# KTH-RPL/cloth-splatting

Hardware: AMD Instinct MI355X
Metric: rasterizer fwd+bwd rendered Mpix/s (scene_1, 800x800) (higher is better)
Workload: dtype f32

## Files before the change

cloth-splatting_amd/csrc/csplat_raster.hip:

```cpp
#include "csplat_common.h"

#include <atomic>
#include <cstring>
#include <chrono>
#include <mutex>
#include <type_traits>

namespace {

constexpr float NEAR_Z = 0.2f;

__device__ constexpr float SH_C0 = 0.28209479177387814f;
__device__ constexpr float SH_C1 = 0.4886025119029199f;
__device__ constexpr float SH_C2[5] = {1.0925484305920792f, -1.0925484305920792f, 0.31539156525252005f,
                                       -1.0925484305920792f, 0.5462742152960396f};
__device__ constexpr float SH_C3[7] = {-0.5900435899266435f, 2.890611442640554f, -0.4570457994644658f,
                                       0.3731763325901154f, -0.4570457994644658f, 1.445305721320277f,
                                       -0.5900435899266435f};

struct Geom {
    float *depth;
    float2 *xy;
    float4 *conic_opacity;
    float *rgb;
// ... 217 lines not shown

    g.depth[i] = depth;
    radii[i] = rad;
    g.xy[i] = make_float2(px, py);
    g.conic_opacity[i] = co;
#pragma unroll
    for (int k = 0; k < 3; k++) g.rgb[3 * i + k] = rgb[k];
#pragma unroll
    for (int k = 0; k < 6; k++) g.cov3D[6 * i + k] = c6[k];
    g.clamped[i] = clampbits;
    g.tiles_touched[i] = touched;
    g.cut2[i] = cut;
    g.pack[3 * (size_t)i] = make_float4(px, py, co.x, co.y);
    g.pack[3 * (size_t)i + 1] = make_float4(co.z, co.w, rgb[0], rgb[1]);
    g.pack[3 * (size_t)i + 2] = make_float4(rgb[2], depth, cut, 0.f);
}

template <bool STAGE>
__global__ __launch_bounds__(256) void k_preprocess(int P, int D, int M, const float *__restrict__ means3D,
                                                     const float *__restrict__ shs,
                                                     const float *__restrict__ colors_precomp,
                                                     const float *__restrict__ opacities,
                                                     const float *__restrict__ scales, float scale_mod,
                                                     const float *__restrict__ rotations,
                                                     const float *__restrict__ cov3D_precomp, Cam cam, Geom g,
                                                     int32_t *__restrict__ radii, int nocull) {
    __shared__ float s_shrows[STAGE ? 256 * SH_ROW : 1];
    if (STAGE) {
        const int base = blockIdx.x * 256;
        stage_sh_rows<256>(shs + (size_t)base * 48, min(256, P - base), s_shrows);
        __syncthreads();
    }
    preprocess_body<STAGE>(P, D, M, means3D, shs, colors_precomp, opacities, scales, scale_mod, rotations, cov3D_precomp, cam, g, radii,
                           nocull, s_shrows, (int)(blockIdx.x * blockDim.x + threadIdx.x), (int)threadIdx.x);
}

constexpr int K1_MAX_VIEWS = 8;
struct K1View {
    const float *means3D, *rotations;
    Cam cam;
    Geom g;
    int32_t *radii;
    uint32_t *table, *info, *mailbox;
    int2 *ranges;
    uint32_t tag;
};
struct K1Table { int n; K1View v[K1_MAX_VIEWS]; };

constexpr int K1V_G = 64;
template <bool STAGE>
__global__ __launch_bounds__(256) void k_preprocess_views(int P, int D, int M, const float *__restrict__ shs,
                                                           const float *__restrict__ opacities,
                                                           const float *__restrict__ scales, float scale_mod, K1Table tab,
                                                           int nocull) {
    __shared__ float s_shrows[STAGE ? K1V_G * SH_ROW : 1];
    const int base = blockIdx.x * K1V_G;
    if (STAGE) {
        stage_sh_rows<256>(shs + (size_t)base * 48, min(K1V_G, P - base), s_shrows);
        __syncthreads();
    }
    const int lane = threadIdx.x & 63;
    for (int vi = threadIdx.x >> 6; vi < tab.n; vi += 4) {
        const K1View &w = tab.v[vi];
        preprocess_body<STAGE>(P, D, M, w.means3D, shs, nullptr, opacities, scales, scale_mod, w.rotations, nullptr, w.cam, w.g, w.radii, nocull,
                               s_shrows, base + lane, lane);
    }
}

__global__ __launch_bounds__(256) void k_emit_keys(int P, const float2 *__restrict__ xy, const float *__restrict__ depth,
                                                    const uint32_t *__restrict__ offsets,
                                                    const int32_t *__restrict__ radii, Cam cam,
                                                    uint64_t *__restrict__ keys, uint32_t *__restrict__ ids) {
    const int i = blockIdx.x * blockDim.x + threadIdx.x;
    if (i >= P) return;
    const int rad = radii[i];
    if (rad <= 0) return;
    uint32_t off = (i == 0) ? 0u : offsets[i - 1];
    const float2 p = xy[i];
    int minx, miny, maxx, maxy;
    tile_rect(p.x, p.y, rad, cam, minx, miny, maxx, maxy);
    const uint32_t dbits = __float_as_uint(depth[i]);
    for (int y = miny; y < maxy; y++)
        for (int x = minx; x < maxx; x++) {
            keys[off] = ((uint64_t)(uint32_t)(y * cam.gx + x) << 32) | dbits;
            ids[off] = (uint32_t)i;
            off++;
        }
}

__global__ __launch_bounds__(256) void k_tile_ranges(int64_t R, const uint64_t *__restrict__ keys, int2 *__restrict__ ranges) {
    const int64_t i = (int64_t)blockIdx.x * blockDim.x + threadIdx.x;
    if (i >= R) return;
    const uint32_t t = (uint32_t)(keys[i] >> 32);
    if (i == 0) ranges[t].x = 0;
    else {
        const uint32_t tp = (uint32_t)(keys[i - 1] >> 32);
        if (tp != t) { ranges[tp].y = (int)i; ranges[t].x = (int)i; }
    }
    if (i == R - 1) ranges[t].y = (int)R;
}

constexpr int BUCKET_CAP = 8192;
constexpr int BUCKET_TILES = 12288;
constexpr int BUCKET_G = 1024;

__device__ __forceinline__ void tile_count_body(int P, int tiles, const float2 *__restrict__ xy,
                                                const int32_t *__restrict__ radii, const Cam &cam,
                                                uint32_t *__restrict__ table) {
    extern __shared__ uint32_t s_hist[];
    for (int t = threadIdx.x; t < tiles; t += BUCKET_G) s_hist[t] = 0u;
    __syncthreads();
    const int i = blockIdx.x * BUCKET_G + threadIdx.x;
    if (i < P) {
        const int rad = radii[i];
        if (rad > 0) {
            const float2 p = xy[i];
            int minx, miny, maxx, maxy;
            tile_rect(p.x, p.y, rad, cam, minx, miny, maxx, maxy);
            for (int y = miny; y < maxy; y++)
                for (int x = minx; x < maxx; x++) atomicAdd(&s_hist[y * cam.gx + x], 1u);
        }
    }
    __syncthreads();
    uint32_t *row = table + (size_t)blockIdx.x * tiles;
    for (int t = threadIdx.x; t < tiles; t += BUCKET_G) row[t] = s_hist[t];
}
__global__ __launch_bounds__(BUCKET_G) void k_tile_count(int P, int tiles, const float2 *__restrict__ xy,
                                                          const int32_t *__restrict__ radii, Cam cam,
                                                          uint32_t *__restrict__ table) {
    tile_count_body(P, tiles, xy, radii, cam, table);
}
__global__ __launch_bounds__(BUCKET_G) void k_tile_count_views(int P, int tiles, K1Table tab) {
    const K1View &w = tab.v[blockIdx.y];
    tile_count_body(P, tiles, w.g.xy, w.radii, w.cam, w.table);
}

__device__ __forceinline__ void tile_colscan_body(int tiles, int nb, uint32_t *__restrict__ table, uint32_t *__restrict__ cnt) {
    const int t = blockIdx.x * 256 + threadIdx.x;
    if (t >= tiles) return;
    uint32_t run = 0;
    int b = 0;
    for (; b + 8 <= nb; b += 8) {
        uint32_t v[8];
#pragma unroll
        for (int u = 0; u < 8; u++) v[u] = table[(size_t)(b + u) * tiles + t];
#pragma unroll
        for (int u = 0; u < 8; u++) { table[(size_t)(b + u) * tiles + t] = run; run += v[u]; }
    }
    for (; b < nb; b++) { const uint32_t v = table[(size_t)b * tiles + t]; table[(size_t)b * tiles + t] = run; run += v; }
    cnt[t] = run;
}
__global__ __launch_bounds__(256) void k_tile_colscan(int tiles, int nb, uint32_t *__restrict__ table, uint32_t *__restrict__ cnt) {
    tile_colscan_body(tiles, nb, table, cnt);
}
__global__ __launch_bounds__(256) void k_tile_colscan_views(int tiles, int nb, K1Table tab) {
    uint32_t *table = tab.v[blockIdx.y].table;
    tile_colscan_body(tiles, nb, table, table + (size_t)nb * tiles);
}

constexpr int INFO_BUSY = 64;
constexpr int LPT_BINS = 512;
__device__ __forceinline__ void tile_scan_body(int tiles, const uint32_t *__restrict__ cnt, int2 *__restrict__ ranges,
                                               uint32_t *__restrict__ info, volatile uint32_t *mailbox, uint32_t tag) {
    __shared__ unsigned long long s_w[17];
    __shared__ uint32_t s_max[16];
    const int lane = threadIdx.x & 63, w = threadIdx.x >> 6;
    unsigned long long carry = 0ull;
    uint32_t mx = 0;
    uint32_t *busy = info + INFO_BUSY;
    for (int base = 0; base < tiles; base += 1024) {
        const int t = base + threadIdx.x;
        const uint32_t c = t < tiles ? cnt[t] : 0u;
        mx = max(mx, c);
        const unsigned long long v0 = (unsigned long long)c | ((unsigned long long)(c ? 1u : 0u) << 32);
        unsigned long long inc = v0;
#pragma unroll
        for (int d = 1; d < 64; d <<= 1) { const unsigned long long o = __shfl_up(inc, d, 64); if (lane >= d) inc += o; }
        if (lane == 63) s_w[w] = inc;
        __syncthreads();
        if (w == 0) {
            unsigned long long v = lane < 16 ? s_w[lane] : 0ull, vi = v;
#pragma unroll
            for (int d = 1; d < 16; d <<= 1) { const unsigned long long o = __shfl_up(vi, d, 64); if (lane >= d) vi += o; }
            if (lane < 16) s_w[lane] = vi - v;
            if (lane == 15) s_w[16] = vi;
        }
        __syncthreads();
        const unsigned long long exl = carry + s_w[w] + inc - v0;
        const uint32_t ex = (uint32_t)exl;
        if (t < tiles) {
            ranges[t] = c ? make_int2((int)ex, (int)(ex + c)) : make_int2(0, 0);
            if (c) busy[1 + (uint32_t)(exl >> 32)] = (uint32_t)t;
            else busy[tiles + 4 + tiles - 1 - (t - (int)(uint32_t)(exl >> 32))] = (uint32_t)t;
        }
        carry += s_w[16];
        __syncthreads();
    }
    {
        __shared__ uint32_t s_bin[LPT_BINS + 1];
        const uint32_t nbusy = (uint32_t)(carry >> 32);
        uint32_t *lpt = busy + tiles + 4;
        for (int i = threadIdx.x; i <= LPT_BINS; i += 1024) s_bin[i] = 0u;
        __syncthreads();
        for (uint32_t i = threadIdx.x; i < nbusy; i += 1024) {
            const uint32_t c = cnt[busy[1 + i]];
            atomicAdd(&s_bin[LPT_BINS - 1 - min(c >> 4, (uint32_t)(LPT_BINS - 1))], 1u);
        }
        __syncthreads();
        if (w == 0) {
            uint32_t v[LPT_BINS / 64], run = 0;
// ... 43 lines not shown

__device__ __forceinline__ void emit_bucket_body(int P, int tiles, const float2 *__restrict__ xy,
                                                 const float *__restrict__ depth, const int32_t *__restrict__ radii,
                                                 const Cam &cam, const uint32_t *__restrict__ table,
                                                 const int2 *__restrict__ ranges, uint64_t *__restrict__ comp) {
    extern __shared__ uint32_t s_base[];
    const uint32_t *row = table + (size_t)blockIdx.x * tiles;
    for (int t = threadIdx.x; t < tiles; t += BUCKET_G) s_base[t] = (uint32_t)ranges[t].x + row[t];
    __syncthreads();
    const int i = blockIdx.x * BUCKET_G + threadIdx.x;
    if (i >= P) return;
    const int rad = radii[i];
    if (rad <= 0) return;
    const float2 p = xy[i];
    int minx, miny, maxx, maxy;
    tile_rect(p.x, p.y, rad, cam, minx, miny, maxx, maxy);
    const uint64_t v = ((uint64_t)__float_as_uint(depth[i]) << 32) | (uint32_t)i;
    for (int y = miny; y < maxy; y++)
        for (int x = minx; x < maxx; x++) comp[atomicAdd(&s_base[y * cam.gx + x], 1u)] = v;
}
__global__ __launch_bounds__(BUCKET_G) void k_emit_bucket(int P, int tiles, const float2 *__restrict__ xy,
                                                           const float *__restrict__ depth, const int32_t *__restrict__ radii,
                                                           Cam cam, const uint32_t *__restrict__ table,
                                                           const int2 *__restrict__ ranges, uint64_t *__restrict__ comp) {
    emit_bucket_body(P, tiles, xy, depth, radii, cam, table, ranges, comp);
}

constexpr int P2_MAX_VIEWS = 8;
struct P2View {
    Geom g;
    Cam cam;
    const int32_t *radii;
    const uint32_t *table;
    int2 *ranges;
    uint64_t *keys_u, *keys_sorted;
    uint32_t *ids_sorted;
    int *seg_offset, *slot_tile;
    float4 *ckpt;
    uint16_t *mask16;
    unsigned long long *bbits;
    unsigned long long *bmask;
    float4 *recA, *recB;
    float2 *recC;
    const float *bg;
    float *final_T;
    uint32_t *n_contrib;
    float *out_color, *out_depth;
    uint32_t R;
    const uint32_t *info;
    uint32_t Lcap;
    uint32_t Bcap;
    int spec;
};
struct P2Table { P2View v[P2_MAX_VIEWS]; uint32_t *valid; int nviews; };
__device__ __forceinline__ bool p2_live(const P2View &w) { return !w.spec || (w.info[0] - 1u < w.R && w.info[1] <= w.Lcap && w.info[2] <= w.Bcap); }
__device__ __forceinline__ void seg_plan_body(int tiles, const int2 *__restrict__ ranges, int *__restrict__ seg_offset,
                                              int *__restrict__ slot_tile);
__global__ __launch_bounds__(BUCKET_G) void k_emit_bucket_views(int P, int tiles, P2Table tab) {
    const P2View &w = tab.v[blockIdx.y];
    if (!p2_live(w)) return;
    if (blockIdx.x == gridDim.x - 1) { seg_plan_body(tiles, w.ranges, w.seg_offset, w.slot_tile); return; }
    emit_bucket_body(P, tiles, w.g.xy, w.g.depth, w.radii, w.cam, w.table, w.ranges, w.keys_u);
}

constexpr int TSORT_THREADS = 1024;
constexpr int TSORT_WAVES = TSORT_THREADS / 64;
constexpr int TSORT_ITEMS = BUCKET_CAP / TSORT_THREADS;
constexpr int TSORT_NB = 4 * TSORT_THREADS;
constexpr int TSORT_GRID = 512;
constexpr int TSORT_LONG = 64;
constexpr int TSORT_WORDS = TSORT_NB + 4 + 256 + 8 + 2 + 2 + TSORT_WAVES + 2;
__host__ __device__ inline size_t tsort_lds_bytes(int longest) {
    const int items = (longest > 0 ? longest : 1) + TSORT_THREADS - 1;
    return (size_t)(items / TSORT_THREADS) * TSORT_THREADS * 8 + (size_t)TSORT_WORDS * 4;
}

__device__ __forceinline__ void tile_sort_body(const int2 *__restrict__ ranges, const uint64_t *__restrict__ comp,
                                               uint64_t *__restrict__ keys_sorted,
                                               uint32_t *__restrict__ ids_sorted, int mode, int tile) {
    extern __shared__ uint64_t s_key[];
    const int2 r = ranges[tile];
    const int n = r.y - r.x;
    if (n <= 0) return;
    const int skip_byte3 = mode & 1;
    const int items = (n + TSORT_THREADS - 1) / TSORT_THREADS;
    uint32_t *s_cnt = reinterpret_cast<uint32_t *>(s_key + (size_t)items * TSORT_THREADS);
    uint32_t *s_dig = s_cnt + TSORT_NB + 4;
    const int lane = threadIdx.x & 63, w = threadIdx.x >> 6;
    const int wbase = w * items * 64;
    const uint64_t lt = (1ull << lane) - 1ull;
    uint64_t key[TSORT_ITEMS];
    uint32_t rank[TSORT_ITEMS];
#pragma unroll
    for (int i = 0; i < TSORT_ITEMS; i++) {
        const int idx = wbase + i * 64 + lane;
        key[i] = (i < items && idx < n) ? comp[r.x + idx] : ~0ull;
    }
    uint32_t *s_diff = s_dig + 264;
    uint32_t *s_mm = s_diff + 2;
    uint32_t *s_wtot = s_mm + 2;
    const uint64_t hi = (uint64_t)(uint32_t)tile << 32;
    if (!(mode & 2)) {
        uint32_t dmin = ~0u, dmax = 0u;
#pragma unroll
        for (int i = 0; i < TSORT_ITEMS; i++) {
            const int idx = wbase + i * 64 + lane;
            if (i < items && idx < n) { const uint32_t d = (uint32_t)(key[i] >> 32); dmin = min(dmin, d); dmax = max(dmax, d); }
// ... 589 lines not shown
        for (int o = 1; o < 16; o <<= 1) m = max(m, (uint32_t)__shfl_xor((int)m, o, 64));
        if (lane == 0) reinterpret_cast<uint32_t *>(seg_offset)[tiles + 1 + tile * 16 + blk] = m;
    }
    if (inside && r == 0) {
        final_T[pix] = T;
        n_contrib[pix] = last;
        const size_t HW = (size_t)H * W;
        out_color[pix] = C0 + T * bg[0];
        out_color[HW + pix] = C1 + T * bg[1];
        out_color[2 * HW + pix] = C2 + T * bg[2];
        out_depth[pix] = Dp;
    }
}
template <int CTRL>
__device__ __forceinline__ float dpp_add(float v) {
    return v + __int_as_float(__builtin_amdgcn_update_dpp(0, __float_as_int(v), CTRL, 0xF, 0xF, false));
}
#define CSPLAT_ROW_SCAN4(OP, N, FIRST, a, b, c, d)                                                                                  \
    asm(FIRST "v_" OP "_f32_dpp %0, %0, %0 row_shr:" #N " row_mask:0xf bank_mask:0xf\n\t"                                          \
              "v_" OP "_f32_dpp %1, %1, %1 row_shr:" #N " row_mask:0xf bank_mask:0xf\n\t"                                          \
              "v_" OP "_f32_dpp %2, %2, %2 row_shr:" #N " row_mask:0xf bank_mask:0xf\n\t"                                          \
              "v_" OP "_f32_dpp %3, %3, %3 row_shr:" #N " row_mask:0xf bank_mask:0xf"                                               \
        : "+v"(a), "+v"(b), "+v"(c), "+v"(d))
__device__ __forceinline__ void row_scan4_mul(float (&x)[4]) {
    CSPLAT_ROW_SCAN4("mul", 1, "s_nop 1\n\t", x[0], x[1], x[2], x[3]);
    CSPLAT_ROW_SCAN4("mul", 2, "", x[0], x[1], x[2], x[3]);
    CSPLAT_ROW_SCAN4("mul", 4, "", x[0], x[1], x[2], x[3]);
    CSPLAT_ROW_SCAN4("mul", 8, "", x[0], x[1], x[2], x[3]);
}
__device__ __forceinline__ void row_scan4_add(float (&x)[4]) {
    CSPLAT_ROW_SCAN4("add", 1, "s_nop 1\n\t", x[0], x[1], x[2], x[3]);
    CSPLAT_ROW_SCAN4("add", 2, "", x[0], x[1], x[2], x[3]);
    CSPLAT_ROW_SCAN4("add", 4, "", x[0], x[1], x[2], x[3]);
    CSPLAT_ROW_SCAN4("add", 8, "", x[0], x[1], x[2], x[3]);
}
__device__ __forceinline__ void row_scan4_min(float (&x)[4]) {
    CSPLAT_ROW_SCAN4("min", 1, "s_nop 1\n\t", x[0], x[1], x[2], x[3]);
    CSPLAT_ROW_SCAN4("min", 2, "", x[0], x[1], x[2], x[3]);
    CSPLAT_ROW_SCAN4("min", 4, "", x[0], x[1], x[2], x[3]);
    CSPLAT_ROW_SCAN4("min", 8, "", x[0], x[1], x[2], x[3]);
}
__device__ __forceinline__ float row_total(float v) {
    v = dpp_add<0xB1>(v); v = dpp_add<0x4E>(v); v = dpp_add<0x141>(v); v = dpp_add<0x140>(v);
    return v;
}
__device__ __forceinline__ void composite_fwd16_body(int tiles, int W, int H, int gx, const int2 *__restrict__ ranges,
                                                     const uint16_t *__restrict__ mask16, const float4 *__restrict__ recA,
                                                     const float4 *__restrict__ recB, const float2 *__restrict__ recC,
                                                     uint32_t null_rec, const float *__restrict__ bg,
                                                     int *seg_offset, float4 *__restrict__ ckpt,
                                                     float *__restrict__ final_T, uint32_t *__restrict__ n_contrib,
                                                     float *__restrict__ out_color, float *__restrict__ out_depth,
                                                     unsigned long long *__restrict__ bbits,
                                                     const unsigned long long *__restrict__ bmask,
                                                     const uint32_t *__restrict__ order = nullptr) {
    __shared__ int s_ring[RING16];
    __shared__ uint32_t s_hit[SEG / 32];
    const int wg = blockIdx.x;
    const int item = ((wg >> 7) << 3) + (wg & 7), blk = (wg >> 3) & 15;
    if (item >= tiles) return;
    const int tile = order ? (int)order[item] : item;
    const int lane = threadIdx.x, sv = lane & 15, q = lane >> 4;
    const int px0 = (tile % gx) * CSPLAT_TILE + (blk & 3) * 4;
    const int py = (tile / gx) * CSPLAT_TILE + (blk >> 2) * 4 + q;
    const float fy = (float)py;
    const int2 range = ranges[tile];
    const int n = range.y - range.x;
    const uint32_t rx = (uint32_t)range.x;
    __shared__ float s_Tend[16];
    bool inside[4];
    unsigned long long m_done[4];
    float T[4], C0[4], C1[4], C2[4], Dp[4], fx[4];
    uint32_t last[4];
#pragma unroll
    for (int j = 0; j < 4; j++) {
        inside[j] = px0 + j < W && py < H;
        m_done[j] = __builtin_amdgcn_ballot_w64(!inside[j]);
        T[j] = inside[j] ? 1.f : 0.f; C0[j] = C1[j] = C2[j] = Dp[j] = 0.f;
        last[j] = 0u;
        fx[j] = (float)(px0 + j);
    }
    int seg0 = 0, seg_written = -1;
    if (n > 0 && (m_done[0] & m_done[1] & m_done[2] & m_done[3]) != ~0ull) {
        seg0 = seg_offset[tile];
        WordStreamT<16, RING16> st;
        st.start(bmask, rx, n, blk, lane, s_ring);
        if (lane < SEG / 32) s_hit[lane] = 0u;
        auto fetch = [&](Trip &t, int k) -> bool {
            const bool ok = st.group(k, sv, t.pos);
            const uint32_t ri = t.pos >= 0 ? rx + (uint32_t)t.pos : null_rec;
            t.a = recA[ri]; t.b = recB[ri]; t.c = recC[ri];
            return ok;
        };
        auto process = [&](const Trip &t) {
            const int seg = __builtin_amdgcn_readfirstlane(t.pos) / SEG;
            if (seg != seg_written) {
#pragma unroll
                for (int j = 0; j < 4; j++) {
                    const float t0 = row_total(C0[j]), t1 = row_total(C1[j]), t2 = row_total(C2[j]);
                    if (sv == 0)
                        for (int s_ = seg_written + 1; s_ <= seg; s_++)
                            ckpt[(size_t)(seg0 + s_) * 256 + blk * 16 + q * 4 + j] = make_float4(T[j], t0, t1, t2);
                    C0[j] = sv == 0 ? t0 : 0.f; C1[j] = sv == 0 ? t1 : 0.f; C2[j] = sv == 0 ? t2 : 0.f;
                }
                if (seg_written >= 0) bbits_flush(s_hit, bbits, (size_t)(seg0 + seg_written), blk, lane);
                for (int s_ = seg_written + 1; s_ < seg; s_++) bbits_zero(bbits, (size_t)(seg0 + s_), blk, lane);
                seg_written = seg;
            }
            const float dy = t.a.y - fy;
            float al[4], inc[4];
            unsigned long long m_live[4];
// ... 81 lines not shown
#pragma unroll
    for (int j = 0; j < 4; j++)
        if (inside[j] && __builtin_amdgcn_inverse_ballot_w64(m_done[j])) T[j] = s_Tend[q * 4 + j];
    uint32_t hi_ = 0u;
#pragma unroll
    for (int j = 0; j < 4; j++) {
        C0[j] = row_total(C0[j]); C1[j] = row_total(C1[j]); C2[j] = row_total(C2[j]); Dp[j] = row_total(Dp[j]);
        uint32_t m = last[j];
#pragma unroll
        for (int o = 1; o < 16; o <<= 1) m = max(m, (uint32_t)__shfl_xor((int)m, o, 64));
        last[j] = m;
        hi_ = max(hi_, inside[j] ? m : 0u);
    }
    {
#pragma unroll
        for (int o = 16; o < 64; o <<= 1) hi_ = max(hi_, (uint32_t)__shfl_xor((int)hi_, o, 64));
        if (lane == 0) reinterpret_cast<uint32_t *>(seg_offset)[tiles + 1 + tile * 16 + blk] = hi_;
    }
    if (sv < 4) {
        const size_t HW = (size_t)H * W;
        float t_ = T[0], c0 = C0[0], c1 = C1[0], c2 = C2[0], dp = Dp[0];
        uint32_t la = last[0];
        bool in_ = inside[0];
#pragma unroll
        for (int j = 1; j < 4; j++)
            if (sv == j) { t_ = T[j]; c0 = C0[j]; c1 = C1[j]; c2 = C2[j]; dp = Dp[j]; la = last[j]; in_ = inside[j]; }
        if (in_) {
            const int pix = py * W + px0 + sv;
            final_T[pix] = t_;
            n_contrib[pix] = la;
            out_color[pix] = c0 + t_ * bg[0];
            out_color[HW + pix] = c1 + t_ * bg[1];
            out_color[2 * HW + pix] = c2 + t_ * bg[2];
            out_depth[pix] = dp;
        }
    }
    if (seg_written >= 0) bbits_flush(s_hit, bbits, (size_t)(seg0 + seg_written), blk, lane);
}
template <bool ROWS>
__global__ __launch_bounds__(64) void k_composite_fwd(int tiles, int W, int H, int gx, const int2 *__restrict__ ranges,
                                                       const uint16_t *__restrict__ mask16, const float4 *__restrict__ recA,
                                                       const float4 *__restrict__ recB, const float2 *__restrict__ recC,
                                                       uint32_t null_rec, const float *__restrict__ bg,
                                                       int *seg_offset, float4 *__restrict__ ckpt,
                                                       float *__restrict__ final_T, uint32_t *__restrict__ n_contrib,
                                                       float *__restrict__ out_color, float *__restrict__ out_depth,
                                                       unsigned long long *__restrict__ bbits,
                                                       const unsigned long long *__restrict__ bmask) {
    if (ROWS)
        composite_fwd_body(tiles, W, H, gx, ranges, mask16, recA, recB, recC, null_rec, bg, seg_offset, ckpt, final_T, n_contrib, out_color,
                           out_depth, (int)blockIdx.x, bbits);
    else
        composite_fwd16_body(tiles, W, H, gx, ranges, mask16, recA, recB, recC, null_rec, bg, seg_offset, ckpt, final_T, n_contrib, out_color,
                             out_depth, bbits, bmask);
}
constexpr int K6_EXTRA = 256;
__device__ __forceinline__ void paint_empty_tiles(int tiles, int W, int H, int gx, const uint32_t *__restrict__ order, int busy_grid,
                                                  const float *__restrict__ bg, int *seg_offset, float *__restrict__ final_T,
                                                  uint32_t *__restrict__ n_contrib, float *__restrict__ out_color,
                                                  float *__restrict__ out_depth) {
    const int lane = threadIdx.x;
    const size_t HW = (size_t)H * W;
    const float b0 = bg[0], b1 = bg[1], b2 = bg[2];
    uint32_t *blk_hi = reinterpret_cast<uint32_t *>(seg_offset) + tiles + 1;
    for (int pos = (busy_grid >> 7 << 3) + ((int)blockIdx.x - busy_grid); pos < tiles; pos += (int)gridDim.x - busy_grid) {
        const int tile = (int)order[pos];
        if (lane < 16) blk_hi[tile * 16 + lane] = 0u;
#pragma unroll
        for (int q = 0; q < 4; q++) {
            const int px = (tile % gx) * CSPLAT_TILE + (lane & 15), py = (tile / gx) * CSPLAT_TILE + 4 * q + (lane >> 4);
            if (px < W && py < H) {
                const int pix = py * W + px;
                final_T[pix] = 1.f;
                n_contrib[pix] = 0u;
                out_color[pix] = b0; out_color[HW + pix] = b1; out_color[2 * HW + pix] = b2;
                out_depth[pix] = 0.f;
            }
        }
    }
}
template <bool ROWS>
__global__ __launch_bounds__(64) __attribute__((amdgpu_waves_per_eu(5))) void k_composite_fwd_views(int tiles, int W, int H, P2Table tab, int busy_grid) {
    if (tab.valid && blockIdx.x == 0 && blockIdx.y == 0 && threadIdx.x == 0) {
        bool ok = true;
        for (int i = 0; i < tab.nviews; i++) ok = ok && p2_live(tab.v[i]);
        *tab.valid = ok ? 1u : 0u;
    }
    const P2View &w = tab.v[blockIdx.y];
    if (!p2_live(w)) return;
    const uint32_t *order = w.info + INFO_BUSY + tiles + 4;
    if ((int)blockIdx.x >= busy_grid) {
        paint_empty_tiles(tiles, W, H, w.cam.gx, order, busy_grid, w.bg, w.seg_offset, w.final_T, w.n_contrib, w.out_color, w.out_depth);
        return;
    }
    if (ROWS)
        composite_fwd_body(tiles, W, H, w.cam.gx, w.ranges, w.mask16, w.recA, w.recB, w.recC, w.R, w.bg, w.seg_offset, w.ckpt, w.final_T,
                           w.n_contrib, w.out_color, w.out_depth, (int)blockIdx.x, w.bbits, order);
    else
        composite_fwd16_body(tiles, W, H, w.cam.gx, w.ranges, w.mask16, w.recA, w.recB, w.recC, w.R, w.bg, w.seg_offset, w.ckpt, w.final_T,
                             w.n_contrib, w.out_color, w.out_depth, w.bbits, w.bmask, order);
}

constexpr int ACC_STRIDE = 16;

#define CSPLAT_ROWMASK_OP(OP, dst, src0, src1, RM)                                                                                  \
    asm("s_nop 1\n\tv_" OP "_f32_dpp %0, %1, %2 quad_perm:[0,1,2,3] row_mask:" RM " bank_mask:0xf" : "+v"(dst) : "v"(src0), "v"(src1))
__device__ __forceinline__ void rows_scan_mul(float f, float Tin, float &Tr, float &Tout) {
    const auto s16 = __builtin_amdgcn_permlane16_swap(__float_as_uint(f), __float_as_uint(f), false, false);
    const float ev = __uint_as_float(s16[0]), od = __uint_as_float(s16[1]);
    const float pr = ev * od;
    const auto s32 = __builtin_amdgcn_permlane32_swap(__float_as_uint(pr), __float_as_uint(pr), false, false);
    const float lo = __uint_as_float(s32[0]), hi = __uint_as_float(s32[1]);
    float base = Tin;
    CSPLAT_ROWMASK_OP("mul", base, lo, Tin, "0xc");
    Tr = base;
    CSPLAT_ROWMASK_OP("mul", Tr, ev, base, "0xa");
    Tout = (Tin * lo) * hi;
}
__device__ __forceinline__ void rows_scan_add(float g, float Sin, float &Sr, float &Sout) {
    const auto s16 = __builtin_amdgcn_permlane16_swap(__float_as_uint(g), __float_as_uint(g), false, false);
    const float ev = __uint_as_float(s16[0]), od = __uint_as_float(s16[1]);
    const float pr = ev + od;
    const auto s32 = __builtin_amdgcn_permlane32_swap(__float_as_uint(pr), __float_as_uint(pr), false, false);
    const float lo = __uint_as_float(s32[0]), hi = __uint_as_float(s32[1]);
    float base = Sin;
    CSPLAT_ROWMASK_OP("add", base, lo, Sin, "0xc");
    float incl = ev;
    CSPLAT_ROWMASK_OP("add", incl, od, ev, "0xa");
    Sr = base + incl;
    Sout = (Sin + lo) + hi;
}
#ifndef CSPLAT_K7X
#define CSPLAT_K7X 0
#endif
constexpr int RING7 = SEG;
template <bool DET, bool DEPTH = false, bool FEAT = false>
__device__ __forceinline__ void composite_bwd_body(int tiles, int W, int H, int gx, const int2 *__restrict__ ranges,
                                                   const uint32_t *__restrict__ ids_sorted,
                                                   const unsigned long long *__restrict__ bbits, const float4 *__restrict__ recA,
                                                   const float4 *__restrict__ recB, const float2 *__restrict__ recC,
                                                   uint32_t null_rec, const int *__restrict__ seg_offset,
                                                   const int *__restrict__ slot_tile, const float4 *__restrict__ ckpt,
                                                   const float *__restrict__ final_T, const uint32_t *__restrict__ n_contrib,
                                                   const float *__restrict__ out_color, const float *__restrict__ dL_dpix,
                                                   float *__restrict__ acc, float *__restrict__ det,
                                                   unsigned long long *stamp = nullptr, int wg = (int)blockIdx.x,
                                                   const float *__restrict__ dL_ddepth = nullptr, const float *__restrict__ dpart = nullptr,
                                                   const float *__restrict__ features = nullptr, int nf = 0,
                                                   const float *__restrict__ dL_dfeat = nullptr, const float *__restrict__ dL_dalpha = nullptr,
                                                   const float *__restrict__ wpart = nullptr) {
    static_assert(!FEAT || DEPTH, "the feature path is instantiated on the depth path");
    constexpr int DS = FEAT ? 16 : (DEPTH ? 10 : 9);
    using TT = std::conditional_t<FEAT, TripF, Trip>;
// ... 1318 lines not shown
        if (stage)
            k_preprocess<true><<<cdiv(P, 256), 256, 0, s>>>(P, t.D, t.M, t.means3D, t.shs, t.colors_precomp, t.opacities, t.scales,
                                                             t.scale_modifier, t.rotations, t.cov3D_precomp, t.cam, t.g, t.radii, nocull_mode());
        else
            k_preprocess<false><<<cdiv(P, 256), 256, 0, s>>>(P, t.D, t.M, t.means3D, t.shs, t.colors_precomp, t.opacities, t.scales,
                                                              t.scale_modifier, t.rotations, t.cov3D_precomp, t.cam, t.g, t.radii, nocull_mode());
        LAUNCH_CHECK();
    }
    if (t.can_bucket) {
        ProfScope ps(PROF_K2, s);
        if (P > 0) {
            k_tile_count<<<nb, BUCKET_G, (size_t)tiles * 4, s>>>(P, tiles, t.g.xy, t.radii, t.cam, t.table);
            LAUNCH_CHECK();
        } else {
            HIP_TRY(hipMemsetAsync(t.table, 0, (size_t)nb * tiles * 4, s));
        }
        uint32_t *tile_cnt = t.table + (size_t)nb * tiles;
        k_tile_colscan<<<cdiv(tiles, 256), 256, 0, s>>>(tiles, nb, t.table, tile_cnt);
        LAUNCH_CHECK();
        k_tile_scan<<<1, 1024, 0, s>>>(tiles, tile_cnt, t.ranges, t.info, t.mb_dev, t.tag);
        LAUNCH_CHECK();
    }
    return 0;
}

static bool begin_views_compatible(int V, const int *tk) {
    if (V < 1 || V > K1_MAX_VIEWS || (g_debug_flags & 512u)) return false;
    const FwdTicket &a = g_tickets[tk[0]];
    if (a.P <= 0 || !a.can_bucket || !a.shs || a.colors_precomp || a.cov3D_precomp || !a.scales || !a.rotations) return false;
    for (int i = 1; i < V; i++) {
        const FwdTicket &w = g_tickets[tk[i]];
        if (w.P != a.P || w.D != a.D || w.M != a.M || w.W != a.W || w.H != a.H || w.shs != a.shs || w.opacities != a.opacities ||
            w.scales != a.scales || w.scale_modifier != a.scale_modifier || w.colors_precomp || w.cov3D_precomp || !w.rotations ||
            !w.can_bucket)
            return false;
    }
    return true;
}
static int begin_launch_views(int V, const int *tk, hipStream_t join) {
    const FwdTicket &a = g_tickets[tk[0]];
    const int P = a.P, tiles = a.tiles, nb = a.nb;
    K1Table tab;
    tab.n = V;
    for (int i = 0; i < V; i++) {
        const FwdTicket &t = g_tickets[tk[i]];
        K1View &k = tab.v[i];
        k.means3D = t.means3D; k.rotations = t.rotations; k.cam = t.cam; k.g = t.g; k.radii = t.radii; k.table = t.table;
        k.info = t.info; k.mailbox = t.mb_dev; k.ranges = t.ranges; k.tag = t.tag;
    }
    {
        ProfScope ps(PROF_K1, join);
        const bool stage = a.M == 16 && ((uintptr_t)a.shs & 15u) == 0;
        if (stage)
            k_preprocess_views<true><<<cdiv(P, K1V_G), 256, 0, join>>>(P, a.D, a.M, a.shs, a.opacities, a.scales, a.scale_modifier, tab,
                                                                     nocull_mode());
        else
            k_preprocess_views<false><<<cdiv(P, K1V_G), 256, 0, join>>>(P, a.D, a.M, a.shs, a.opacities, a.scales, a.scale_modifier, tab,
                                                                      nocull_mode());
        LAUNCH_CHECK();
    }
    {
        ProfScope ps(PROF_K2, join);
        k_tile_count_views<<<dim3(nb, V), BUCKET_G, (size_t)tiles * 4, join>>>(P, tiles, tab);
        LAUNCH_CHECK();
        k_tile_colscan_views<<<dim3(cdiv(tiles, 256), V), 256, 0, join>>>(tiles, nb, tab);
        LAUNCH_CHECK();
        k_tile_scan_views<<<V, 1024, 0, join>>>(tiles, nb, tab);
        LAUNCH_CHECK();
    }
    return 0;
}

int csplat_forward_begin(void *stream, int P, int D, int M, const float *bg, int W, int H, const float *means3D,
                         const float *shs, const float *colors_precomp, const float *opacities, const float *scales,
                         float scale_modifier, const float *rotations, const float *cov3D_precomp, const float *view,
                         const float *proj, const float *campos, float tanfovx, float tanfovy, int prefiltered,
                         csplat_alloc_fn alloc, void *alloc_ctx, int32_t *radii, int *ticket_out) {
    if (int rc = begin_prepare(stream, P, D, M, bg, W, H, means3D, shs, colors_precomp, opacities, scales, scale_modifier, rotations,
                               cov3D_precomp, view, proj, campos, tanfovx, tanfovy, prefiltered, alloc, alloc_ctx, radii, ticket_out))
        return rc;
    const int rc = begin_launch(g_tickets[*ticket_out]);
    if (rc) {
        std::lock_guard<std::mutex> lk(g_ticket_mu);
        g_tickets[*ticket_out].used = false;
    }
    return rc;
}

static int finish_read(const FwdTicket &t, uint32_t host_info[3], hipStream_t launched_on = nullptr) {
    hipStream_t s = launched_on ? launched_on : t.s;
    host_info[0] = host_info[1] = host_info[2] = 0;
    if (t.can_bucket) {
        bool got = false;
        if (t.use_mail) {
            const auto t0 = std::chrono::steady_clock::now();
            unsigned spins = 0;
            while (!(got = (t.mb_host[2] == t.tag))) {
                if ((++spins & 0x3FFu) == 0 &&
                    std::chrono::duration<double>(std::chrono::steady_clock::now() - t0).count() > 2.0) break;
            }
            if (got) { host_info[0] = t.mb_host[0]; host_info[1] = t.mb_host[1]; host_info[2] = t.mb_host[3]; }
        }
        if (!got) {
            HIP_TRY(hipMemcpyAsync(host_info, t.info, 12, hipMemcpyDeviceToHost, s));
            HIP_TRY(hipStreamSynchronize(s));
        }
    } else if (t.P > 0) {
        ProfScope ps(PROF_K2, s);
        if (int rc = csplat_inclusive_scan_u32(s, t.g.tiles_touched, t.g.offsets, t.P, t.g.scan_tmp)) return rc;
        HIP_TRY(hipMemcpyAsync(host_info, t.g.offsets + (t.P - 1), 4, hipMemcpyDeviceToHost, s));
        HIP_TRY(hipStreamSynchronize(s));
        host_info[1] = 0xFFFFFFFFu;
        host_info[2] = 0xFFFFFFFFu;
    }
    CSPLAT_REQUIRE(host_info[0] <= 0x7FFFFFFFu, "csplat_forward: more than 2^31 - 1 tile instances (Gaussian x tile pairs) in one view");
    return 0;
}
static uint32_t tile_sort_cap() {
// ... 30 lines not shown
        P2Table tab;
        tab.valid = valid; tab.nviews = V;
        uint32_t maxR = 0;
        for (int i = 0; i < V; i++) {
            const FwdTicket &t = g_tickets[tk[i]];
            const uint32_t R = Rcap[i];
            maxR = R > maxR ? R : maxR;
            void *bbase = t.alloc(t.alloc_ctx, CSPLAT_CHUNK_BINNING, csplat_binning_bytes(R, W, H));
            void *tbase = t.alloc(t.alloc_ctx, CSPLAT_CHUNK_TEMP, csplat_temp_bytes(P, R, W, H));
            CSPLAT_REQUIRE(bbase && tbase, "allocator returned NULL");
            size_t boff[B_NFIELDS], toff[5];
            binning_offsets(R, tiles, boff);
            temp_offsets(R, toff);
            P2View &k = tab.v[i];
            k.g = t.g; k.cam = t.cam; k.radii = t.radii; k.table = t.table; k.ranges = t.ranges;
            k.keys_u = (uint64_t *)((char *)tbase + toff[0]);
            k.keys_sorted = (uint64_t *)((char *)bbase + boff[0]);
            k.ids_sorted = (uint32_t *)((char *)bbase + boff[1]);
            k.seg_offset = (int *)((char *)bbase + boff[2]);
            k.slot_tile = (int *)((char *)bbase + boff[3]);
            k.ckpt = (float4 *)((char *)bbase + boff[4]);
            k.mask16 = (uint16_t *)((char *)bbase + boff[5]);
            k.bbits = (unsigned long long *)((char *)bbase + boff[9]);
            k.bmask = (unsigned long long *)((char *)bbase + boff[10]);
            k.recA = (float4 *)((char *)bbase + boff[6]); k.recB = (float4 *)((char *)bbase + boff[7]);
            k.recC = (float2 *)((char *)bbase + boff[8]);
            k.bg = t.bg; k.final_T = t.final_T; k.n_contrib = t.n_contrib; k.out_color = v[i].out_color; k.out_depth = v[i].out_depth;
            k.R = R; k.info = t.info; k.Lcap = Lcap; k.Bcap = Bcap; k.spec = spec;
            v[i].layout_rendered = (int)R; v[i].geom = t.gbase; v[i].binning = bbase; v[i].image = t.ibase;
        }
        {
            ProfScope ps(PROF_K3, join);
            k_emit_bucket_views<<<dim3(nb + 1, V), BUCKET_G, (size_t)tiles * 4, join>>>(P, tiles, tab);
            LAUNCH_CHECK();
        }
        {
            const size_t lds = tsort_lds_bytes((int)Lcap);
            ProfScope ps(PROF_K4, join);
            k_tile_sort_views<<<dim3(tiles < TSORT_GRID ? tiles : TSORT_GRID, V), TSORT_THREADS, lds, join>>>(tab, tsort_mode(P));
            LAUNCH_CHECK();
        }
        {
            ProfScope ps(PROF_K5, join);
            const int exact = (g_debug_flags & (1u | 16u | 32u)) ? 0 : 1, nbm = cdiv((int64_t)maxR + 1, 256);
            if (V == 1 || V == 2 || V == 4 || V == 8)
                k_block_masks_views<<<dim3((unsigned)(((int64_t)nbm * V + 7) / 8 * 8)), 256, 0, join>>>(tab, exact, V);
            else
                k_block_masks_views<<<dim3(nbm, V), 256, 0, join>>>(tab, exact, 0);
            LAUNCH_CHECK();
        }
        {
            ProfScope ps(PROF_K6, join);
            const int total = cdiv(tiles, 8) * 128, bg_ = cdiv((int)Bcap, 8) * 128, busy_grid = bg_ < total ? bg_ : total;
            if (!(g_debug_flags & 32768u))
                k_composite_fwd_views<false><<<dim3(busy_grid + K6_EXTRA, V), 64, 0, join>>>(tiles, W, H, tab, busy_grid);
            else
                k_composite_fwd_views<true><<<dim3(busy_grid + K6_EXTRA, V), 64, 0, join>>>(tiles, W, H, tab, busy_grid);
            LAUNCH_CHECK();
        }
        return 0;
    }
}

static int finish_views_batched(int V, const int *tk, csplat_view *v, hipStream_t join, bool *done, int mode = 0,
                                PendingViews *pend = nullptr, int *relaunched = nullptr) {
    *done = false;
    if (V < 1 || V > P2_MAX_VIEWS || (g_debug_flags & 512u)) return 0;
    const FwdTicket &a = g_tickets[tk[0]];
    for (int i = 0; i < V; i++) {
        const FwdTicket &t = g_tickets[tk[i]];
        if (!t.can_bucket || t.P != a.P || t.W != a.W || t.H != a.H || t.P <= 0) return 0;
    }
    const int P = a.P, W = a.W, H = a.H, tiles = a.tiles;
    const uint32_t cap = tile_sort_cap();
    uint32_t info[P2_MAX_VIEWS][3];
    bool have_info = false;
    auto read_counts = [&]() -> int {
        for (int i = 0; i < V && !have_info; i++)
            if (int rc = finish_read(g_tickets[tk[i]], info[i], join)) return rc;
        have_info = true;
        return 0;
    };
    auto launch = [&](const uint32_t *Rcap, uint32_t Lcap, int spec, uint32_t Bcap) -> int { return p2_launch(V, tk, v, join, Rcap, Lcap, spec, Bcap); };
    auto remember = [&]() {
        std::lock_guard<std::mutex> lk(g_spec_mu);
        SpecHist &e = g_spec_ring[g_spec_next];
        g_spec_next = (g_spec_next + 1) % SPEC_RING;
        e.W = W; e.H = H; e.P = P; e.R = 0; e.longest = 0; e.busy = 0;
        for (int i = 0; i < V; i++) {
            e.R = info[i][0] > e.R ? info[i][0] : e.R;
            e.longest = info[i][1] > e.longest ? info[i][1] : e.longest;
            e.busy = info[i][2] > e.busy ? info[i][2] : e.busy;
        }
    };
    auto release = [&]() {
        std::lock_guard<std::mutex> lk(g_ticket_mu);
        for (int i = 0; i < V; i++) g_tickets[tk[i]].used = false;
    };
    SpecHist hist;
    {
        std::lock_guard<std::mutex> lk(g_spec_mu);
        for (const SpecHist &e : g_spec_ring)
            if (e.R > 0 && e.W == W && e.H == H && e.P == P) {
                hist.W = W; hist.H = H; hist.P = P;
                hist.R = e.R > hist.R ? e.R : hist.R;
                hist.longest = e.longest > hist.longest ? e.longest : hist.longest;
                hist.busy = e.busy > hist.busy ? e.busy : hist.busy;
            }
    }
    if (mode == 2 || (!(g_debug_flags & 1024u) && hist.R > 0)) {
// ... 962 lines not shown
```

Baseline: 4563.

## Replace tile column-scan kernel with atomic offsets and interleave K6 views

```diff
diff --git a/cloth-splatting_amd/csrc/csplat_raster.hip b/cloth-splatting_amd/csrc/csplat_raster.hip
--- a/cloth-splatting_amd/csrc/csplat_raster.hip
+++ b/cloth-splatting_amd/csrc/csplat_raster.hip
@@ -293,7 +293,12 @@
 __global__ __launch_bounds__(256) void k_preprocess_views(int P, int D, int M, const float *__restrict__ shs,
                                                            const float *__restrict__ opacities,
                                                            const float *__restrict__ scales, float scale_mod, K1Table tab,
-                                                           int nocull) {
+                                                           int nocull, int tiles, int nb) {
+    if ((int)blockIdx.x * K1V_G >= P) {
+        for (int vi = 0; vi < tab.n; vi++)
+            for (int t = threadIdx.x; t < tiles; t += 256) tab.v[vi].table[(size_t)nb * tiles + t] = 0u;
+        return;
+    }
     __shared__ float s_shrows[STAGE ? K1V_G * SH_ROW : 1];
     const int base = blockIdx.x * K1V_G;
     if (STAGE) {
@@ -347,7 +352,7 @@
 
 __device__ __forceinline__ void tile_count_body(int P, int tiles, const float2 *__restrict__ xy,
                                                 const int32_t *__restrict__ radii, const Cam &cam,
-                                                uint32_t *__restrict__ table) {
+                                                uint32_t *__restrict__ table, uint32_t *__restrict__ tot = nullptr) {
     extern __shared__ uint32_t s_hist[];
     for (int t = threadIdx.x; t < tiles; t += BUCKET_G) s_hist[t] = 0u;
     __syncthreads();
@@ -364,16 +369,23 @@
     }
     __syncthreads();
     uint32_t *row = table + (size_t)blockIdx.x * tiles;
-    for (int t = threadIdx.x; t < tiles; t += BUCKET_G) row[t] = s_hist[t];
+    if (tot) {
+        for (int t = threadIdx.x; t < tiles; t += BUCKET_G) {
+            const uint32_t c = s_hist[t];
+            row[t] = c ? atomicAdd(&tot[t], c) : 0u;
+        }
+    } else {
+        for (int t = threadIdx.x; t < tiles; t += BUCKET_G) row[t] = s_hist[t];
+    }
 }
 __global__ __launch_bounds__(BUCKET_G) void k_tile_count(int P, int tiles, const float2 *__restrict__ xy,
                                                           const int32_t *__restrict__ radii, Cam cam,
                                                           uint32_t *__restrict__ table) {
     tile_count_body(P, tiles, xy, radii, cam, table);
 }
-__global__ __launch_bounds__(BUCKET_G) void k_tile_count_views(int P, int tiles, K1Table tab) {
+__global__ __launch_bounds__(BUCKET_G) void k_tile_count_views(int P, int tiles, int nb, K1Table tab) {
     const K1View &w = tab.v[blockIdx.y];
-    tile_count_body(P, tiles, w.g.xy, w.radii, w.cam, w.table);
+    tile_count_body(P, tiles, w.g.xy, w.radii, w.cam, w.table, w.table + (size_t)nb * tiles);
 }
 
 __device__ __forceinline__ void tile_colscan_body(int tiles, int nb, uint32_t *__restrict__ table, uint32_t *__restrict__ cnt) {
@@ -393,10 +405,6 @@
 }
 __global__ __launch_bounds__(256) void k_tile_colscan(int tiles, int nb, uint32_t *__restrict__ table, uint32_t *__restrict__ cnt) {
     tile_colscan_body(tiles, nb, table, cnt);
-}
-__global__ __launch_bounds__(256) void k_tile_colscan_views(int tiles, int nb, K1Table tab) {
-    uint32_t *table = tab.v[blockIdx.y].table;
-    tile_colscan_body(tiles, nb, table, table + (size_t)nb * tiles);
 }
 
 constexpr int INFO_BUSY = 64;
@@ -546,7 +554,14 @@
     uint32_t Bcap;
     int spec;
 };
-struct P2Table { P2View v[P2_MAX_VIEWS]; uint32_t *valid; int nviews; };
+struct P2Table {
+    P2View v[P2_MAX_VIEWS];
+    uint32_t *valid;
+    int nviews;
+#ifdef CSPLAT_K6_STAMPS
+    unsigned long long *k6_stamp;
+#endif
+};
 __device__ __forceinline__ bool p2_live(const P2View &w) { return !w.spec || (w.info[0] - 1u < w.R && w.info[1] <= w.Lcap && w.info[2] <= w.Bcap); }
 __device__ __forceinline__ void seg_plan_body(int tiles, const int2 *__restrict__ ranges, int *__restrict__ seg_offset,
                                               int *__restrict__ slot_tile);
@@ -1242,11 +1257,10 @@
                                                      float *__restrict__ final_T, uint32_t *__restrict__ n_contrib,
                                                      float *__restrict__ out_color, float *__restrict__ out_depth,
                                                      unsigned long long *__restrict__ bbits,
-                                                     const unsigned long long *__restrict__ bmask,
+                                                     const unsigned long long *__restrict__ bmask, int wg,
                                                      const uint32_t *__restrict__ order = nullptr) {
     __shared__ int s_ring[RING16];
     __shared__ uint32_t s_hit[SEG / 32];
-    const int wg = blockIdx.x;
     const int item = ((wg >> 7) << 3) + (wg & 7), blk = (wg >> 3) & 15;
     if (item >= tiles) return;
     const int tile = order ? (int)order[item] : item;
@@ -1434,10 +1448,11 @@
                            out_depth, (int)blockIdx.x, bbits);
     else
         composite_fwd16_body(tiles, W, H, gx, ranges, mask16, recA, recB, recC, null_rec, bg, seg_offset, ckpt, final_T, n_contrib, out_color,
-                             out_depth, bbits, bmask);
+                             out_depth, bbits, bmask, (int)blockIdx.x);
 }
 constexpr int K6_EXTRA = 256;
-__device__ __forceinline__ void paint_empty_tiles(int tiles, int W, int H, int gx, const uint32_t *__restrict__ order, int busy_grid,
+static_assert(K6_EXTRA % 128 == 0, "a view's K6 waves are whole 128-wave groups");
+__device__ __forceinline__ void paint_empty_tiles(int tiles, int W, int H, int gx, const uint32_t *__restrict__ order, int busy_grid, int x,
                                                   const float *__restrict__ bg, int *seg_offset, float *__restrict__ final_T,
                                                   uint32_t *__restrict__ n_contrib, float *__restrict__ out_color,
                                                   float *__restrict__ out_depth) {
@@ -1445,7 +1460,7 @@
     const size_t HW = (size_t)H * W;
     const float b0 = bg[0], b1 = bg[1], b2 = bg[2];
     uint32_t *blk_hi = reinterpret_cast<uint32_t *>(seg_offset) + tiles + 1;
-    for (int pos = (busy_grid >> 7 << 3) + ((int)blockIdx.x - busy_grid); pos < tiles; pos += (int)gridDim.x - busy_grid) {
+    for (int pos = (busy_grid >> 7 << 3) + (x - busy_grid); pos < tiles; pos += K6_EXTRA) {
         const int tile = (int)order[pos];
         if (lane < 16) blk_hi[tile * 16 + lane] = 0u;
 #pragma unroll
@@ -1461,26 +1476,48 @@
         }
     }
 }
+#ifdef CSPLAT_K6_STAMPS
+struct K6Stamp {
+    unsigned long long *p = nullptr;
+    __device__ K6Stamp(unsigned long long *buf, size_t pos, int view, int x, int busy_grid, int tiles, const P2View &w, const uint32_t *order) {
+        if (!buf || threadIdx.x != 0) return;
+        p = buf + pos * 4;
+        const unsigned long long t0 = __builtin_amdgcn_s_memrealtime();
+        __builtin_amdgcn_s_waitcnt(0xC07F);
+        const int item = ((x >> 7) << 3) + (x & 7);
+        long long n = -1;
+        if (x < busy_grid && item < tiles) { const int2 r = w.ranges[order[item]]; n = r.y - r.x; }
+        p[0] = t0; p[2] = (unsigned long long)(view | (x << 8)); p[3] = (unsigned long long)n;
+    }
+    __device__ ~K6Stamp() {
+        if (p) { const unsigned long long t1 = __builtin_amdgcn_s_memrealtime(); __builtin_amdgcn_s_waitcnt(0xC07F); p[1] = t1; }
+    }
+};
+#endif
 template <bool ROWS>
 __global__ __launch_bounds__(64) __attribute__((amdgpu_waves_per_eu(5))) void k_composite_fwd_views(int tiles, int W, int H, P2Table tab, int busy_grid) {
-    if (tab.valid && blockIdx.x == 0 && blockIdx.y == 0 && threadIdx.x == 0) {
+    if (tab.valid && blockIdx.x == 0 && threadIdx.x == 0) {
         bool ok = true;
         for (int i = 0; i < tab.nviews; i++) ok = ok && p2_live(tab.v[i]);
         *tab.valid = ok ? 1u : 0u;
     }
-    const P2View &w = tab.v[blockIdx.y];
+    const int grp = (int)blockIdx.x >> 7, view = grp % tab.nviews, x = ((grp / tab.nviews) << 7) | ((int)blockIdx.x & 127);
+    const P2View &w = tab.v[view];
     if (!p2_live(w)) return;
     const uint32_t *order = w.info + INFO_BUSY + tiles + 4;
-    if ((int)blockIdx.x >= busy_grid) {
-        paint_empty_tiles(tiles, W, H, w.cam.gx, order, busy_grid, w.bg, w.seg_offset, w.final_T, w.n_contrib, w.out_color, w.out_depth);
+#ifdef CSPLAT_K6_STAMPS
+    K6Stamp stamp_(tab.k6_stamp, blockIdx.x, view, x, busy_grid, tiles, w, order);
+#endif
+    if (x >= busy_grid) {
+        paint_empty_tiles(tiles, W, H, w.cam.gx, order, busy_grid, x, w.bg, w.seg_offset, w.final_T, w.n_contrib, w.out_color, w.out_depth);
         return;
     }
     if (ROWS)
         composite_fwd_body(tiles, W, H, w.cam.gx, w.ranges, w.mask16, w.recA, w.recB, w.recC, w.R, w.bg, w.seg_offset, w.ckpt, w.final_T,
-                           w.n_contrib, w.out_color, w.out_depth, (int)blockIdx.x, w.bbits, order);
+                           w.n_contrib, w.out_color, w.out_depth, x, w.bbits, order);
     else
         composite_fwd16_body(tiles, W, H, w.cam.gx, w.ranges, w.mask16, w.recA, w.recB, w.recC, w.R, w.bg, w.seg_offset, w.ckpt, w.final_T,
-                             w.n_contrib, w.out_color, w.out_depth, w.bbits, w.bmask, order);
+                             w.n_contrib, w.out_color, w.out_depth, w.bbits, w.bmask, x, order);
 }
 
 constexpr int ACC_STRIDE = 16;
@@ -2905,18 +2942,16 @@
         ProfScope ps(PROF_K1, join);
         const bool stage = a.M == 16 && ((uintptr_t)a.shs & 15u) == 0;
         if (stage)
-            k_preprocess_views<true><<<cdiv(P, K1V_G), 256, 0, join>>>(P, a.D, a.M, a.shs, a.opacities, a.scales, a.scale_modifier, tab,
-                                                                     nocull_mode());
+            k_preprocess_views<true><<<cdiv(P, K1V_G) + 1, 256, 0, join>>>(P, a.D, a.M, a.shs, a.opacities, a.scales, a.scale_modifier, tab,
+                                                                     nocull_mode(), tiles, nb);
         else
-            k_preprocess_views<false><<<cdiv(P, K1V_G), 256, 0, join>>>(P, a.D, a.M, a.shs, a.opacities, a.scales, a.scale_modifier, tab,
-                                                                      nocull_mode());
+            k_preprocess_views<false><<<cdiv(P, K1V_G) + 1, 256, 0, join>>>(P, a.D, a.M, a.shs, a.opacities, a.scales, a.scale_modifier, tab,
+                                                                      nocull_mode(), tiles, nb);
         LAUNCH_CHECK();
     }
     {
         ProfScope ps(PROF_K2, join);
-        k_tile_count_views<<<dim3(nb, V), BUCKET_G, (size_t)tiles * 4, join>>>(P, tiles, tab);
-        LAUNCH_CHECK();
-        k_tile_colscan_views<<<dim3(cdiv(tiles, 256), V), 256, 0, join>>>(tiles, nb, tab);
+        k_tile_count_views<<<dim3(nb, V), BUCKET_G, (size_t)tiles * 4, join>>>(P, tiles, nb, tab);
         LAUNCH_CHECK();
         k_tile_scan_views<<<V, 1024, 0, join>>>(tiles, nb, tab);
         LAUNCH_CHECK();
@@ -3053,10 +3088,14 @@
         {
             ProfScope ps(PROF_K6, join);
             const int total = cdiv(tiles, 8) * 128, bg_ = cdiv((int)Bcap, 8) * 128, busy_grid = bg_ < total ? bg_ : total;
+            const unsigned grid = (unsigned)(busy_grid + K6_EXTRA) * (unsigned)V;
+#ifdef CSPLAT_K6_STAMPS
+            tab.k6_stamp = csplat_stamp_buffer((size_t)grid * 4);
+#endif
             if (!(g_debug_flags & 32768u))
-                k_composite_fwd_views<false><<<dim3(busy_grid + K6_EXTRA, V), 64, 0, join>>>(tiles, W, H, tab, busy_grid);
+                k_composite_fwd_views<false><<<grid, 64, 0, join>>>(tiles, W, H, tab, busy_grid);
             else
-                k_composite_fwd_views<true><<<dim3(busy_grid + K6_EXTRA, V), 64, 0, join>>>(tiles, W, H, tab, busy_grid);
+                k_composite_fwd_views<true><<<grid, 64, 0, join>>>(tiles, W, H, tab, busy_grid);
             LAUNCH_CHECK();
         }
         return 0;
```

After: 4713 (median of 6 runs). 1.03x the previous value.
